# atom501/v-img

Measured on AMD Instinct MI355X. Metric: Mrays/sec (primary+secondary) at 512 spp, higher is better.
Workload: dtype f32; 1 GPU; disney_spheres.json, mis integrator, 512 spp, 1800x800; integrator=mis, spp=512, depth=unbounded, bvh=sweep SAH (host)

## Files before the change

v-img_amd/csrc/hip_internal.h:

```cpp
#pragma once
#include <hip/hip_runtime.h>

#include <algorithm>
#include <string>
#include <utility>
#include <vector>

#include "../../include/vimg_hip.h"
#include "device_mem.h"
#include "device_scene.h"
#include "kernel_tus.h"

#pragma GCC visibility push(hidden)
struct VimgDeviceScene {
  vimg::DScene d{};
  vimg::DevBuf nodes, leaf_prims;
  vimg::DevBuf chain_leaf;
  std::vector<vimg::DevBuf> tables;
  size_t total_bytes = 0;
  bool textured = false;
  VimgHipOptions opt{};
  int waves_per_simd = 2;
  bool too_wide = false;
  bool force_general = false;
  bool no_lds_tables = false;
  uint32_t num_cus = 0;
  uint32_t num_leaf_prims = 0;
  vimg::DevBuf stats;
  vimg::DevBuf counter;
  vimg::DevBuf root_box;
  vimg::DevBuf frame;
  vimg::DevBuf pool_cold;
  vimg::DevBuf stack_ovf;
  vimg::DevBuf pool_state;
  uint32_t pool_epoch = 0;
  uint64_t generation = 0;
  uint32_t num_vertices = 0, num_tris = 0, num_spheres = 0;
  uint32_t num_meshes = 0;
  std::vector<std::pair<uint32_t, uint32_t>> normal_rows;
  uint32_t n_internal = 0;
// ... 111 lines not shown
};
int enqueue_render(VimgDeviceScene* s, const VimgRenderParams* p, const RenderLaunch& r);
int check_kernel_error(VimgDeviceScene* s);
uint64_t fetch_shard_pixels(const VimgDeviceScene* s, const VimgRenderParams* p);
int fetch_stats(VimgDeviceScene* s, const VimgRenderParams* p, VimgRenderStats* out);

LaunchCfg make_launch(const VimgDeviceScene* s, const VimgRenderParams* p, int sx, int sy);
LaunchCfg make_launch_lane(const VimgDeviceScene* s, const VimgRenderParams* p, int sx, int sy);
LaunchCfg make_launch_feature(const VimgDeviceScene* s, const VimgRenderParams* p, int sx, int sy);
RenderArgs base_args(const VimgDeviceScene* s, const VimgRenderParams* p, int sx, int sy);
uint32_t segments_for(const VimgDeviceScene* s, const VimgRenderParams* p, uint64_t items, uint64_t in_flight,
                      double per_gen, double most, RenderArgs* a);
const void* kernel_of(const VimgDeviceScene* s, const LaunchCfg& c);
const void* launched_kernel_of(const VimgDeviceScene* s, const LaunchCfg& c, bool stats);
bool plain_launch_serves(const VimgDeviceScene* s, const LaunchCfg& c, bool stats);
void drop_unread_tables(const VimgDeviceScene* s, LaunchCfg& c, bool stats);

}
#pragma GCC visibility pop
```

v-img_amd/csrc/kernel_tus.h:

```cpp
#pragma once
#include "device_scene.h"

namespace vimg {

struct CuKArgs;
using RenderKernel = void (*)(const DScene, const RenderArgs, float*, DeviceStats*, unsigned int*);
using CuKernel = void (*)(const CuKArgs);

RenderKernel vimg_lane_kernel(bool tex, int wps);
RenderKernel vimg_feature_kernel(bool tex);
CuKernel vimg_cu_kernel(bool tex, bool deep, int nw);
CuKernel vimg_cu_kernel_early(bool tex, bool deep, int nw);
CuKernel vimg_cu_kernel_diag(bool tex, bool deep, int nw);
CuKernel vimg_cu_kernel_plain();
CuKernel vimg_cu_kernel_plain_early();

}
```

v-img_amd/csrc/launch_policy.hip:

```cpp
#include <cmath>

#include "hip_internal.h"
#include "render_cu_kernel.h"

namespace vimg {

uint32_t local_tiles(const VimgDeviceScene* s, const VimgRenderParams* p) {
  const uint32_t total = tiles_of(s->d.res_x) * tiles_of(s->d.res_y);
  if (p->tile_rank >= total) return 0;
  return (total - p->tile_rank + p->tile_world - 1) / p->tile_world;
}

RenderArgs base_args(const VimgDeviceScene* s, const VimgRenderParams* p, int sx, int sy) {
  const VimgHipOptions& o = s->opt;
  RenderArgs a{};
  a.integrator = p->integrator;
  a.samples = p->samples;
  a.spp_div = static_cast<float>(p->samples);
  a.depth = p->depth;
  a.tile_rank = p->tile_rank;
  a.tile_world = p->tile_world;
  a.tiles_x = tiles_of(s->d.res_x);
  a.tiles_y = tiles_of(s->d.res_y);
  a.num_local_tiles = local_tiles(s, p);
// ... 15 lines not shown
  const double gens = double(items) / double(in_flight);
  uint32_t k = gens >= 10.0 ? 1u : uint32_t(std::min(most, std::max(1.0, std::floor(per_gen / gens + 0.5))));
  k = std::min<uint32_t>(k, std::max<uint32_t>(p->samples / 4u, 1u));
  if (items * 2u < in_flight * 3u) k = 1u;
  if (s->opt.pool_segments != VIMG_OPT_AUTO) k = uint32_t(std::max(1, s->opt.pool_segments));
  k = std::min<uint32_t>(k, 4096u);
  while (k > 1u && items * k >= 0xfff00000ull) --k;
  const uint32_t len = std::max<uint32_t>((p->samples + k - 1) / k, 1u);
  a->pool_seg_len = len;
  a->pool_segments = std::max<uint32_t>((p->samples + len - 1) / len, 1u);
  return len;
}

namespace {

CuKernel pick_cu_kernel(const VimgDeviceScene* s, bool deep, int nw, bool diag = false, bool early = false, bool plain = false) {
  if (plain) return early ? vimg_cu_kernel_plain_early() : vimg_cu_kernel_plain();
  return diag ? vimg_cu_kernel_diag(s->textured, deep, nw)
              : (early ? vimg_cu_kernel_early(s->textured, deep, nw) : vimg_cu_kernel(s->textured, deep, nw));
}

void magic_div(uint32_t d, uint32_t* magic, uint32_t* shift) {
  uint32_t l = 0;
  while ((1ull << l) < d) ++l;
  *magic = static_cast<uint32_t>((1ull << (31u + l)) / d + 1ull);
  *shift = l - 1u;
}

constexpr uint32_t CU_LDS_LIMIT = 160u * 1024u;

LaunchCfg cu_launch_with(const VimgDeviceScene* s, const VimgRenderParams* p, int sx, int sy, uint32_t node_budget, uint32_t stack_cap) {
  LaunchCfg c{};
// ... 130 lines not shown
void cu_scratch(const VimgDeviceScene* s, LaunchCfg& c) {
  const RenderArgs& a = c.args;
  c.cold_bytes = size_t(c.grid) * cu_cold_records(s->textured) * a.pool_slots * 16u;
  if (a.stack_lds < a.stack_entries)
    c.ovf_bytes = size_t(c.grid) * a.cu_walkers * (a.stack_entries - a.stack_lds) * 256u;
}

}

const void* kernel_of(const VimgDeviceScene* s, const LaunchCfg& c) {
  if (c.feature) return reinterpret_cast<const void*>(vimg_feature_kernel(s->textured));
  if (c.sched == VIMG_SCHED_CU) return reinterpret_cast<const void*>(pick_cu_kernel(s, c.deep, c.cu_waves));
  return reinterpret_cast<const void*>(vimg_lane_kernel(s->textured, c.wps));
}

bool plain_launch_serves(const VimgDeviceScene* s, const LaunchCfg& c, bool stats) {
  return plain_build_serves(plain_launch_of(c.sched == VIMG_SCHED_CU, s->textured, c.deep, c.cu_waves, stats, s->force_general, c.args)) &&
         plain_tables_serve(c.args.lds_tables) && plain_leaf_perm_serves(c.args.leaf_perm);
}

void drop_unread_tables(const VimgDeviceScene* s, LaunchCfg& c, bool stats) {
  if (c.sched != VIMG_SCHED_CU || (c.args.lds_tables == 0u && c.args.leaf_perm == 0u) || plain_launch_serves(s, c, stats)) return;
  c.lds_bytes -= c.table_bytes;
  c.table_bytes = 0u;
  c.args.lds_tables = 0u;
  c.args.leaf_perm = 0u, c.args.leaf_perm_off = 0u, c.args.leaf_perm_stride = 0u;
}

const void* launched_kernel_of(const VimgDeviceScene* s, const LaunchCfg& c, bool stats) {
  if (c.sched != VIMG_SCHED_CU) return kernel_of(s, c);
  return reinterpret_cast<const void*>(pick_cu_kernel(s, c.deep, c.cu_waves, stats, (c.args.cu_flex & 32u) != 0u,
                                                      plain_launch_serves(s, c, stats)));
}

namespace {

LaunchCfg lane_shaped_launch(const VimgDeviceScene* s, const VimgRenderParams* p, int sx, int sy, bool feature) {
  LaunchCfg c{};
  c.feature = feature;
  const VimgHipOptions& o = s->opt;
  const uint64_t items = (sx >= 0) ? 1 : uint64_t(local_tiles(s, p)) * 64u;
  c.sched = VIMG_SCHED_LANE;
  c.wps = s->waves_per_simd;
  if (o.waves_per_simd != VIMG_OPT_AUTO) c.wps = o.waves_per_simd >= 3 ? 3 : 2;
  RenderArgs& a = c.args = base_args(s, p, sx, sy);
  a.stack_lds = a.stack_entries;
  const uint32_t stack_bytes = 4u * a.stack_entries * 64u * 4u;
// ... 62 lines not shown
```

v-img_amd/csrc/plain_build.h:

```cpp
#pragma once
#include <cstdint>

namespace vimg {

enum : uint32_t {
  PF_INTEGRATOR = 1u,
  PF_CLASSES = 2u,
  PF_LEAF_LDS = 4u,
  PF_SINGLE = 8u,
  PF_ITEMS = 16u,
  PF_FLEX = 32u,
  PF_TAB_HIT = 64u,
  PF_TAB_MAT = 128u,
  PF_TABLES = PF_TAB_HIT | PF_TAB_MAT,
  PF_LEAF_PERM = 256u,
};
#ifdef VIMG_PLAIN_FOLD
constexpr uint32_t PLAIN_FOLD = VIMG_PLAIN_FOLD;
#else
constexpr uint32_t PLAIN_FOLD = PF_INTEGRATOR | PF_CLASSES | PF_LEAF_LDS | PF_SINGLE | PF_ITEMS | PF_FLEX | PF_TAB_HIT | PF_LEAF_PERM;
#endif

struct PlainLaunch {
  bool cu_sched;
  bool textured, deep;
  int cu_waves;
  bool stats;
  bool force_general;
  uint32_t integrator, pool_classes, lds_leaf, cu_flex;
  int single_x;
  bool has_item_list;
};
constexpr uint32_t PLAIN_INTEGRATOR_MIS = 3u;
constexpr uint32_t PLAIN_FLEX_DEFAULT = 1u;

constexpr bool plain_build_serves(const PlainLaunch& l, uint32_t fold = PLAIN_FOLD) {
  if (l.force_general || !l.cu_sched || l.textured || l.deep || l.cu_waves != 16 || l.stats) return false;
  if ((fold & PF_INTEGRATOR) && l.integrator != PLAIN_INTEGRATOR_MIS) return false;
  if ((fold & PF_CLASSES) && l.pool_classes != 3u) return false;
  if ((fold & PF_LEAF_LDS) && l.lds_leaf == 0u) return false;
  if ((fold & PF_SINGLE) && l.single_x >= 0) return false;
  if ((fold & PF_ITEMS) && l.has_item_list) return false;
  if ((fold & PF_FLEX) && (l.cu_flex & ~32u) != PLAIN_FLEX_DEFAULT) return false;
  return true;
}

constexpr bool plain_tables_serve(uint32_t staged, uint32_t fold = PLAIN_FOLD) {
  return (staged & fold & PF_TABLES) == (fold & PF_TABLES);
}

constexpr bool plain_leaf_perm_serves(uint32_t ready, uint32_t fold = PLAIN_FOLD) {
  return !(fold & PF_LEAF_PERM) || ready != 0u;
}

template <class Args>
constexpr PlainLaunch plain_launch_of(bool cu_sched, bool textured, bool deep, int cu_waves, bool stats, bool force_general,
                                      const Args& a) {
  return PlainLaunch{cu_sched, textured, deep, cu_waves, stats || a.full_stats != 0u, force_general,
                     a.integrator, a.pool_classes, a.lds_leaf, a.cu_flex, a.single_x, a.item_list != nullptr};
}

}
```

v-img_amd/csrc/render_cu_kernel.h:

```cpp
#pragma once
#include <type_traits>

#include "plain_build.h"
#include "render_kernels.h"

namespace vimg {

enum : uint32_t {
  SC_THROUGHPUT = 0,
  SC_RESULT,
  SC_NEE,
  SC4_RNG,
  SC4_MAIN
};
__host__ __device__ constexpr uint32_t cu_cold_records(bool tex) { return SC4_MAIN + 1u + (tex ? 1u : 0u); }
__host__ __device__ constexpr uint32_t cu_stack_rows_of(uint32_t entries, uint32_t in_lds) { return in_lds < entries ? in_lds + 1u : entries; }
constexpr uint32_t SLOT_IDLE = 0xffffffffu;

VD void state_store(VIMG_GLOBAL uint32_t* p, uint32_t v) {
  __hip_atomic_store(p, v, __ATOMIC_RELAXED, __HIP_MEMORY_SCOPE_AGENT);
}
VD uint32_t state_load(VIMG_GLOBAL uint32_t* p) {
  return __hip_atomic_load(p, __ATOMIC_RELAXED, __HIP_MEMORY_SCOPE_AGENT);
}
// ... 39 lines not shown
  unsigned long long w_cyc[4];
  unsigned long long wait_cyc[5], wait_n[5];
  unsigned long long ray_cyc, ray_n;
  unsigned long long pv_cyc[6], pv_n;
};
static_assert(sizeof(CuWaveRec) == 416, "CuWaveRec layout");
__host__ __device__ constexpr uint32_t cu_pool_bytes(uint32_t slots, uint32_t waves) {
  return CU_LDS_BYTES * slots + uint32_t(sizeof(CuCtl)) + waves * uint32_t(sizeof(CuWaveRec));
}
VD uint32_t cu_mod(uint32_t n, uint32_t d, uint32_t magic, uint32_t shift) { return n - d * (__umulhi(n, magic) >> shift); }
VD int32_t lds_add_rtn(VIMG_LDS int32_t* p, int32_t v) { return __hip_atomic_fetch_add(p, v, __ATOMIC_RELAXED, __HIP_MEMORY_SCOPE_WORKGROUP); }
VD uint32_t lds_add_rtn(VIMG_LDS uint32_t* p, uint32_t v) { return __hip_atomic_fetch_add(p, v, __ATOMIC_RELAXED, __HIP_MEMORY_SCOPE_WORKGROUP); }
VD uint32_t lds_load(VIMG_LDS uint32_t* p) { return __hip_atomic_load(p, __ATOMIC_RELAXED, __HIP_MEMORY_SCOPE_WORKGROUP); }
VD int32_t lds_load(VIMG_LDS int32_t* p) { return __hip_atomic_load(p, __ATOMIC_RELAXED, __HIP_MEMORY_SCOPE_WORKGROUP); }
VD uint32_t cu_uni(uint32_t v) { return static_cast<uint32_t>(__builtin_amdgcn_readfirstlane(static_cast<int>(v))); }

static_assert(PLAIN_INTEGRATOR_MIS == uint32_t(VIMG_INTEGRATOR_MIS), "plain_build.h");
template <uint32_t PLAIN> VD uint32_t opt_integrator(const RenderArgs& A) {
  if constexpr (PLAIN & PF_INTEGRATOR) return uint32_t(VIMG_INTEGRATOR_MIS); else return A.integrator;
}
template <uint32_t PLAIN> VD uint32_t opt_classes(const RenderArgs& A) {
  if constexpr (PLAIN & PF_CLASSES) return 3u; else return A.pool_classes;
}
template <uint32_t PLAIN> VD bool opt_leaf_in_lds(const RenderArgs& A) {
  if constexpr (PLAIN & PF_LEAF_LDS) return true; else return A.lds_leaf != 0u;
}
template <uint32_t PLAIN> VD bool opt_single(const RenderArgs& A) {
  if constexpr (PLAIN & PF_SINGLE) return false; else return A.single_x >= 0;
}
template <uint32_t PLAIN> VD bool opt_has_items(const RenderArgs& A) {
  if constexpr (PLAIN & PF_ITEMS) return false; else return A.item_list != nullptr;
}
template <uint32_t PLAIN> VD uint32_t opt_flex(const RenderArgs& A) {
  if constexpr (PLAIN & PF_FLEX) return PLAIN_FLEX_DEFAULT; else return A.cu_flex;
}
template <uint32_t PLAIN> constexpr bool opt_leaf_perm = (PLAIN & PF_LEAF_PERM) != 0u;

template <class T>
VD void stage_rows(VIMG_LDS unsigned char* lds_raw, const RenderArgs& A, uint32_t t, gptr<T> src) {
  constexpr uint32_t src_w = uint32_t(sizeof(T)) / 4u;
  const uint32_t dst_w = tab_row_bytes(t) / 4u, words = A.tab_rows[t] * src_w;
  VIMG_LDS uint32_t* dst = reinterpret_cast<VIMG_LDS uint32_t*>(lds_raw + A.tab_off[t]);
  gptr<uint32_t> w = reinterpret_cast<gptr<uint32_t>>(src);
  for (uint32_t i = threadIdx.x; i < words; i += blockDim.x) {
    const uint32_t r = i / src_w;
    dst[r * dst_w + (i - r * src_w)] = w[i];
  }
}
VD void stage_tables(const DScene& g, const RenderArgs& A, VIMG_LDS unsigned char* lds_raw) {
  if (A.lds_tables & PF_TAB_HIT) {
// ... 117 lines not shown
                                         \
  [[maybe_unused]] auto slot_complete = [&](uint32_t nw) -> bool {                                                      \
    return (nw & CF_DONE_V) && (!(nw & CF_HAS_S) || (nw & CF_DONE_S)) && (!(nw & CF_HAS_R) || (nw & CF_DONE_R));        \
  };                                                                                                                    \
    \
  [[maybe_unused]] auto hand_to_vertex = [&](bool complete, uint32_t nw, uint32_t slot_) {                              \
    uint32_t cls_ = 0;                                                                                                  \
    if (complete && (nw & CF_FOUND) && !(nw & CF_KILL_R) && opt_integrator<PLAIN>(A) >= VIMG_INTEGRATOR_MATERIAL) {     \
      cls_ = (nw >> CF_CLS_SHIFT) & 3u;                                                                                 \
      if (cls_ == 0 && material_mode) cls_ = 3;                            \
      if (cls_ != 0) {                                                                                                  \
        if (opt_classes<PLAIN>(A) == 1) cls_ = 1;                                                                       \
        else if (opt_classes<PLAIN>(A) == 2) cls_ = (cls_ == 2) ? 2u : 1u;                                              \
      }                                                                                                                 \
    }                                                                                                                   \
    const unsigned long long m0_ = __ballot(complete && cls_ == 0), m1_ = __ballot(complete && cls_ == 1),              \
                             m2_ = __ballot(complete && cls_ == 2), m3_ = __ballot(complete && cls_ == 3);              \
    if ((m0_ | m1_ | m2_ | m3_) == 0ull) return;                                                                        \
    const uint32_t n_me_ = static_cast<uint32_t>(__popcll(lane == 0 ? m0_ : (lane == 1 ? m1_ : (lane == 2 ? m2_ : m3_)))); \
    uint32_t t_me_ = 0;                                                                                                 \
    if (lane < 4u && n_me_ != 0u) {                                                                                     \
      t_me_ = lds_add_rtn(&G->tail[lane], n_me_);                                                                       \
      if (t_me_ > 0x7ff00000u) raise(8u);                                                                               \
    }                                                                                                                   \
    const uint32_t t0_ = __shfl(t_me_, 0), t1_ = __shfl(t_me_, 1), t2_ = __shfl(t_me_, 2), t3_ = __shfl(t_me_, 3);      \
    if (complete) {                                                                                                     \
      const uint32_t tt_ = cls_ == 0 ? t0_ : (cls_ == 1 ? t1_ : (cls_ == 2 ? t2_ : t3_));                               \
      const unsigned long long mm_ = cls_ == 0 ? m0_ : (cls_ == 1 ? m1_ : (cls_ == 2 ? m2_ : m3_));                     \
      *ring_at(cls_, tt_ + lane_rank(mm_, lane)) = static_cast<uint16_t>(slot_);                                        \
      if (full_stats) tq[slot_] = static_cast<uint32_t>(__builtin_readcyclecounter());                                  \
    }                                                                                                                   \
    __builtin_amdgcn_fence(__ATOMIC_RELEASE, "workgroup");                                                              \
    if (lane < 4u && n_me_ != 0u) lds_add_rtn(&G->avail[lane], static_cast<int32_t>(n_me_));                            \
  };                                                                                                                    \
                     \
  [[maybe_unused]] auto push_rays = [&](bool is_s, bool is_r, uint32_t slot_) {                                         \
    const unsigned long long ms_ = __ballot(is_s), mr_ = __ballot(is_r);                                                \
    const uint32_t n_s_ = static_cast<uint32_t>(__popcll(ms_)), n_r_ = static_cast<uint32_t>(__popcll(mr_));            \
    if (n_s_ + n_r_ == 0u) return;                                                                                      \
    uint32_t t_ = 0;                                                                                                    \
    if (lane == 0) {                                                                                                    \
      t_ = lds_add_rtn(&G->tail[CQ_WALK], n_s_ + n_r_);                                                                 \
      if (t_ > 0x7ff00000u) raise(8u);                                                                                  \
    }                                                                                                                   \
    t_ = cu_uni(t_);                                                                                                    \
    if (is_s) *ring_at(CQ_WALK, t_ + lane_rank(ms_, lane)) = static_cast<uint16_t>(slot_ | CU_RAY_S);                   \
    if (is_r) *ring_at(CQ_WALK, t_ + n_s_ + lane_rank(mr_, lane)) = static_cast<uint16_t>(slot_);                       \
    __builtin_amdgcn_fence(__ATOMIC_RELEASE, "workgroup");                                                              \
// ... 672 lines not shown
        const float root = slab(load3k(g.root_min), load3k(g.root_max), ray.o, w_inv, ray.min_t, ray.max_t);
        cur = is_inf(root) ? REF_DONE : g.root_ref;
        sp = 0;
        w_found = false;
        rec.prim = 0xffffffffu;
        w_setup = false;
      }
    }
    wlap(wc0);
    if (__ballot(w_slot != SLOT_IDLE) == 0ull) break;

    const bool exact_round = __any(w_exact && w_slot != SLOT_IDLE);
    for (;;) {
      auto box_loop = [&](auto exact_possible) {
        for (;;) {
          const bool act = cur != REF_DONE && ref_count(cur) == 0;
          if (!__any(act)) break;
          if (full_stats) d_box += 1u, d_boxl += static_cast<uint32_t>(__popcll(__ballot(act)));
          if (act) {
            v4f na, nb, nc;
            v2u refs;
            if (!DEEP || cur < L.n_nodes) {
              na = L.na[cur], nb = L.nb[cur], nc = L.nc[cur];
              refs = L.nm[cur];
            } else {
              gptr<DNode> nd = g.nodes + cur;
              na = nd->a, nb = nd->b, nc = nd->c;
              refs = v2u{nd->left_ref, nd->right_ref};
            }
            const uint32_t sp_below = sp != 0 ? sp - 1 : 0u;
            uint32_t popped = stack0[(DEEP ? (sp_below < S ? sp_below : S) : sp_below) * 64];
            c_internal += stat_inc;
            float h1, h2;
            if (decltype(exact_possible)::value && w_exact) {
// ... 3 lines not shown
              h1 = slab_fast(f3{na.x, na.y, na.z}, f3{na.w, nb.x, nb.y}, ray.o, w_inv, ray.min_t, ray.max_t);
              h2 = slab_fast(f3{nb.z, nb.w, nc.x}, f3{nc.y, nc.z, nc.w}, ray.o, w_inv, ray.min_t, ray.max_t);
            }
            const bool in1 = !is_inf(h1), in2 = !is_inf(h2);
            const uint32_t c1 = refs.x, c2 = refs.y;
            const bool both = in1 && in2, any = in1 || in2;
            const bool first_is_near = w_any ? false : (h2 > h1);
            const uint32_t near_c = first_is_near ? c1 : c2;
            const uint32_t far_c = first_is_near ? c2 : c1;
            stack0[(DEEP ? (sp < S ? sp : S) : sp) * 64] = far_c;
            if constexpr (DEEP) {
              if (both && sp >= S) ovf0[(sp - S) * 64] = far_c;
              if (!any && sp_below >= S) popped = ovf0[(sp_below - S) * 64];
            }
            const uint32_t one_c = in1 ? c1 : c2;
            cur = both ? near_c : (any ? one_c : (sp != 0 ? popped : REF_DONE));
            sp = both ? sp + 1 : (any ? sp : sp_below);
          }
          if constexpr (DEEP) {
            if (static_cast<uint32_t>(__popcll(__ballot(cur != REF_DONE && ref_count(cur) == 0))) < box_min) break;
          }
        }
      };
      if (exact_round)
        box_loop(std::true_type{});
      else
        box_loop(std::false_type{});
      wlap(wc1);

      if (full_stats) d_leaf += 1u, d_leafl += static_cast<uint32_t>(__popcll(__ballot(cur != REF_DONE && (!DEEP || ref_count(cur) != 0))));
      if (cur != REF_DONE && (!DEEP || ref_count(cur) != 0)) {
        const uint32_t first = ref_index(cur), count = ref_count(cur);
        c_leaf += stat_inc;
        bool stop = false;
        [[maybe_unused]] const VIMG_LDS v4f* leaf0 =
// ... 32 lines not shown
          rec.e2 = keep_rec ? e2 : rec.e2, rec.inv_det = keep_rec ? idet : rec.inv_det;
          rec.prim = keep_rec ? lp_prim : rec.prim;
          rec.kind = keep_rec ? kind : rec.kind;
          w_cls = keep_rec ? lp_cls : w_cls;
          stop = hit && w_any;
        }
        const uint32_t sp_below = sp != 0 ? sp - 1 : 0u;
        uint32_t popped = stack0[(DEEP ? (sp_below < S ? sp_below : S) : sp_below) * 64];
        if constexpr (DEEP) {
          if (!stop && sp_below >= S) popped = ovf0[(sp_below - S) * 64];
        }
        cur = (stop || sp == 0) ? REF_DONE : popped;
        sp = sp_below;
      }
      wlap(wc2);
      const uint32_t n_fin = static_cast<uint32_t>(__popcll(__ballot(w_slot != SLOT_IDLE && cur == REF_DONE)));
      const uint32_t n_act = static_cast<uint32_t>(__popcll(__ballot(w_slot != SLOT_IDLE && cur != REF_DONE)));
      if (n_act == 0 || n_fin >= A.pool_refill) break;
    }

    {
      const bool done = w_slot != SLOT_IDLE && cur == REF_DONE;
      bool complete = false;
      uint32_t nw = 0;
      if (done) {
        uint32_t orv;
        if (w_type == 0u) {
          orv = CF_DONE_S | (w_found ? CF_OCCLUDED : 0u);
        } else {
          orv = CF_DONE_R;
          if (w_found) {
            orv |= CF_FOUND | (rec.kind == 1 ? CF_KIND_SPHERE : 0u) | (w_cls << CF_CLS_SHIFT);
            wr(CR_HIT, w_slot, v4u{fu(rec.e0), fu(rec.e1), fu(rec.e2), fu(rec.inv_det)});
// ... 67 lines not shown
  uint32_t polls = 0;
  unsigned long long idle_since = 0;
  for (;;) {
    const CuKPtr K = cu_kargs();
    CU_STAGE_LOCALS(K);
    auto lap = [&](uint32_t k) {
      if (full_stats) {
        const unsigned long long now = __builtin_readcyclecounter();
        if (lane == 0) wrec->cyc[k] += now - t_mark;
        t_mark = now;
      }
    };
    if (cu_uni(lds_load(&G->abort)) != 0u) break;
    const v4u av4 = *reinterpret_cast<VIMG_LDS v4u*>(&G->avail[0]);
    const int32_t a0 = skip_fin ? 0 : static_cast<int32_t>(cu_uni(av4.x)), a1 = static_cast<int32_t>(cu_uni(av4.y)),
                  a2 = static_cast<int32_t>(cu_uni(av4.z)), a3 = static_cast<int32_t>(cu_uni(av4.w));
    const int32_t aw = static_cast<int32_t>(cu_uni(static_cast<uint32_t>(lds_load(&G->avail[CQ_WALK]))));
    const int32_t m01 = a0 > a1 ? a0 : a1, m23 = a2 > a3 ? a2 : a3, qmax = m01 > m23 ? m01 : m23;
    if (full_stats && lane == 0) {
      wrec->looks += 1;
      wrec->q_sum[0] += static_cast<uint32_t>(a0 > 0 ? a0 : 0), wrec->q_sum[1] += static_cast<uint32_t>(a1 > 0 ? a1 : 0);
      wrec->q_sum[2] += static_cast<uint32_t>(a2 > 0 ? a2 : 0), wrec->q_sum[3] += static_cast<uint32_t>(aw > 0 ? aw : 0);
    }
    if (can_walk && aw > 0 && (aw >= static_cast<int32_t>(A.cu_join) || polls >= A.cu_patience)) {
      lap(5);
      skip_fin = false, polls = 0, idle_since = 0;
      if (full_stats) iter_wave++;
      if (opt_flex<PLAIN>(A) & 4u) __builtin_amdgcn_s_setprio(1);
      cu_walk<TEX, DEEP, NW, DIAG, PLAIN>(n_closest, n_shadow);
      if (opt_flex<PLAIN>(A) & 4u) __builtin_amdgcn_s_setprio(0);
      lap(4);
// ... 12 lines not shown
      lap(5);
      if (full_stats) iter_wave++;
      if (full_stats && lane == 0) wrec->nbatch[cls] += 1, wrec->nslots[cls] += n;
      if (full_stats) {
        unsigned long long w = lane < n ? static_cast<unsigned long long>(static_cast<uint32_t>(__builtin_readcyclecounter()) - tq[e]) : 0ull;
        for (int o = 32; o; o >>= 1) w += __shfl_xor(w, o);
        if (lane == 0) wrec->wait_cyc[cls] += w, wrec->wait_n[cls] += n;
      }
      bool all_pending = false;
      const bool by_class = opt_classes<PLAIN>(A) == 3u;
      if (opt_flex<PLAIN>(A) & 2u) __builtin_amdgcn_s_setprio(1);
      if (cls == 0u)
        cu_vertex<TEX, NW, DIAG, EARLY, true, -1, PLAIN>(n, e, all_pending, n_nan, n_dead);
      else if (cls == 1u && by_class)
        cu_vertex<TEX, NW, DIAG, EARLY, false, int(VIMG_MAT_LAMBERTIAN), PLAIN>(n, e, all_pending, n_nan, n_dead);
      else if (cls == 2u && by_class)
        cu_vertex<TEX, NW, DIAG, EARLY, false, int(VIMG_MAT_PRINCIPLED), PLAIN>(n, e, all_pending, n_nan, n_dead);
      else
        cu_vertex<TEX, NW, DIAG, EARLY, false, -1, PLAIN>(n, e, all_pending, n_nan, n_dead);
      if (opt_flex<PLAIN>(A) & 2u) __builtin_amdgcn_s_setprio(0);
      skip_fin = all_pending;
      if (!all_pending) polls = 0, idle_since = 0;
      lap(cls);
      continue;
    }
    if (cu_uni(lds_load(&G->live)) == 0u) break;
    skip_fin = false;
    polls += 1;
    if ((polls & 255u) == 0u) {
      const unsigned long long now = __builtin_amdgcn_s_memrealtime();
      if (idle_since == 0) idle_since = now;
      else if (static_cast<uint32_t>((now - idle_since) >> 20) > A.cu_watchdog) {
        if (lane == 0) raise(1u);
// ... 45 lines not shown
```

v-img_amd/csrc/render_kernels.h:

```cpp
#pragma once
#include "device_math.h"
#include "device_scene.h"
#include "material_terms.h"
#include "plain_build.h"

namespace vimg {


struct Rng {
  uint64_t s;
};
VD uint32_t pcg_next(Rng& r) {
  uint64_t old = r.s;
  r.s = old * 6364136223846793005ULL + 1ULL;
  uint32_t xorshifted = static_cast<uint32_t>(((old >> 18u) ^ old) >> 27u);
  uint32_t rot = static_cast<uint32_t>(old >> 59u);
  return (xorshifted >> rot) | (xorshifted << ((0u - rot) & 31u));
}
VD void pcg_seed(Rng& r, uint64_t initstate) {
  r.s = 0;
  pcg_next(r);
  r.s += initstate;
  pcg_next(r);
}
// ... 354 lines not shown
  f3 p2t = tri_vertex<PERMUTED>(p2, o, rc.kz);
  p0t.x += rc.sx * p0t.z;
  p0t.y += rc.sy * p0t.z;
  p1t.x += rc.sx * p1t.z;
  p1t.y += rc.sy * p1t.z;
  p2t.x += rc.sx * p2t.z;
  p2t.y += rc.sy * p2t.z;
  float e0 = diff_of_products(p1t.x, p2t.y, p1t.y, p2t.x);
  float e1 = diff_of_products(p2t.x, p0t.y, p2t.y, p0t.x);
  float e2 = diff_of_products(p0t.x, p1t.y, p0t.y, p1t.x);
  if (e0 == 0.f || e1 == 0.f || e2 == 0.f) {
    e0 = diff_of_products_double(p1t.x, p2t.y, p1t.y, p2t.x);
    e1 = diff_of_products_double(p2t.x, p0t.y, p2t.y, p0t.x);
    e2 = diff_of_products_double(p0t.x, p1t.y, p0t.y, p1t.x);
  }
  const bool mixed = (e0 < 0 || e1 < 0 || e2 < 0) && (e0 > 0 || e1 > 0 || e2 > 0);
  const float det = e0 + e1 + e2;
  const float t_scaled = e0 * (p0t.z * rc.sz) + e1 * (p1t.z * rc.sz) + e2 * (p2t.z * rc.sz);
  const float hi = ray.max_t * det, lo = ray.min_t * det;
  const bool out_neg = det < 0 && (t_scaled >= 0 || t_scaled < hi || t_scaled > lo);
  const bool out_pos = det > 0 && (t_scaled <= 0 || t_scaled > hi || t_scaled < lo);
  const bool hit = !mixed && !(det == 0) && !out_neg && !out_pos;
  if (hit) {
    const float inv_det = 1.f / det;
    t_out = t_scaled * inv_det;
    e0o = e0, e1o = e1, e2o = e2, inv_det_o = inv_det;
  }
  return hit;
}
VD bool tri_test_flat(f3 p0, f3 p1, f3 p2, const TravRay& ray, const TriRayConst& rc, float& t_out,
                      float& e0o, float& e1o, float& e2o, float& inv_det_o) {
  return tri_test_body<false>(p0, p1, p2, ray.o, ray, rc, t_out, e0o, e1o, e2o, inv_det_o);
}
VD bool tri_test_permuted(f3 p0, f3 p1, f3 p2, f3 o_perm, const TravRay& ray, const TriRayConst& rc, float& t_out,
                          float& e0o, float& e1o, float& e2o, float& inv_det_o) {
  return tri_test_body<true>(p0, p1, p2, o_perm, ray, rc, t_out, e0o, e1o, e2o, inv_det_o);
}
// ... 1431 lines not shown
```

v-img_amd/csrc/scene_bake.h:

```cpp
#pragma once
#include "device_scene.h"

namespace vimg {

#define VHD static __host__ __device__ __forceinline__

VHD void tri_cross21(const float* v, float c21[3]) {
  const float e1[3] = {v[3] - v[0], v[4] - v[1], v[5] - v[2]};
  const float e2[3] = {v[6] - v[0], v[7] - v[1], v[8] - v[2]};
  c21[0] = e2[1] * e1[2] - e1[1] * e2[2];
  c21[1] = e2[2] * e1[0] - e1[2] * e2[0];
  c21[2] = e2[0] * e1[1] - e1[0] * e2[1];
}

VHD void bake_tri_normal_pdf(const float* v, float n[3], float* area_pdf) {
  const float e1[3] = {v[3] - v[0], v[4] - v[1], v[5] - v[2]};
  const float e2[3] = {v[6] - v[0], v[7] - v[1], v[8] - v[2]};
  const float c12[3] = {e1[1] * e2[2] - e2[1] * e1[2], e1[2] * e2[0] - e2[2] * e1[0],
                        e1[0] * e2[1] - e2[0] * e1[1]};
  const float inv_len = 1.0f / __builtin_sqrtf(c12[0] * c12[0] + c12[1] * c12[1] + c12[2] * c12[2]);
  for (int a = 0; a < 3; ++a) n[a] = c12[a] * inv_len;
  float c21[3];
  tri_cross21(v, c21);
  const float area = __builtin_sqrtf(c21[0] * c21[0] + c21[1] * c21[1] + c21[2] * c21[2]) / 2.0f;
// ... 14 lines not shown
}

VHD void bake_light_tri(const DTriShade& ts, float area_pdf, DLight& L) {
  L.a = v4f{ts.p[0], ts.p[1], ts.p[2], ts.p[3]};
  L.b = v4f{ts.p[4], ts.p[5], ts.p[6], ts.p[7]};
  L.c = v4f{ts.p[8], ts.n[0], ts.n[1], ts.n[2]};
  L.d.w = area_pdf;
}
VHD void bake_light_sphere(const VimgSphere& sp, DLight& L) {
  L.a = v4f{sp.center[0], sp.center[1], sp.center[2], sp.radius};
}

VHD uint32_t bake_material_class(uint32_t type) {
  return type == VIMG_MAT_DIFFUSE_LIGHT ? 0u : type == VIMG_MAT_LAMBERTIAN ? 1u : type == VIMG_MAT_PRINCIPLED ? 2u : 3u;
}
VHD uint32_t bake_material_flags(const VimgMaterial& m, const VimgTexture* textures) {
  uint32_t f = 0;
  if (m.type == VIMG_MAT_PRINCIPLED) f |= MATF_NEEDS_FRAME;
  if (m.tex >= 0 && textures[m.tex].type != VIMG_TEX_CONST) f |= MATF_NEEDS_UV;
  if (m.mr_tex >= 0 || m.normal_map >= 0) f |= MATF_NEEDS_UV;
  return f;
}
VHD uint32_t bake_prim_material(const VimgPrim& p, const DTriShade* shade, const VimgMesh* meshes, const VimgSphere* spheres) {
  return p.type == VIMG_PRIM_TRIANGLE ? meshes[shade[p.index].mesh].material : spheres[p.index].material;
}
VHD DLight bake_light(const VimgLight& l, const VimgPrim* prims, const DTriShade* shade, const float* area_pdf, const VimgMesh* meshes,
                      const VimgSphere* spheres, const VimgMaterial* materials) {
  DLight L{};
  if (l.type == VIMG_LIGHT_BACKGROUND) {
    L.kind = 0u;
// ... 31 lines not shown
```

v-img_amd/csrc/scene_relight.hip:

```cpp
#include <hip/hip_runtime.h>

#include <cstring>

#include "device_math.h"
#include "hip_internal.h"
#include "material_terms.h"
#include "scene_bake.h"

namespace vimg {

namespace {

constexpr uint32_t kBlock = 256;

template <typename T>
VD T* flat(gptr<T> p) {
  return (T*)p;
}

dim3 blocks_for(uint32_t n) { return dim3((n + kBlock - 1) / kBlock); }

}

__global__ void __launch_bounds__(kBlock) scene_relight_flags(const DScene d, uint32_t num_materials) {
// ... 149 lines not shown
      HIP_TRY(hipMemcpyAsync(plan->new_lights.p, u->lights, size_t(u->num_lights) * sizeof(VimgLight), hipMemcpyHostToDevice, st));
      hipLaunchKernelGGL(scene_relight_lights, blocks_for(u->num_lights), dim3(kBlock), 0, st, d, plan->new_lights.as<const VimgLight>(),
                         u->num_lights, plan->new_dlights.as<DLight>());
    }
  } else if (u->materials && d.num_lights) {
    hipLaunchKernelGGL(scene_relight_lights, blocks_for(d.num_lights), dim3(kBlock), 0, st, d, (const VimgLight*)d.lights, d.num_lights,
                       (DLight*)d.dlights);
  }
  HIP_TRY(hipGetLastError());
  return VIMG_OK;
}

void commit_relight(VimgDeviceScene* s, const VimgGeometryUpdate* u, RelightPlan* plan) {
  DScene& d = s->d;
  if (u->textures) s->textures.assign(u->textures, u->textures + s->textures.size());
  if (u->materials) s->materials.assign(u->materials, u->materials + s->materials.size());
  if (u->background) {
    d.background = *u->background;
    d.background_emissive = background_is_emissive(d.background);
  }
  if (plan->new_dmaterials.p) {
    DevBuf& dmaterials = s->tables[s->dmaterials_table];
    dmaterials = std::move(plan->new_dmaterials);
    d.dmaterials = (decltype(d.dmaterials))dmaterials.p;
  }
  s->textured = tables_textured(s->materials.data(), static_cast<uint32_t>(s->materials.size()), s->textures.data(), d.background);
  if (u->set_lights) {
    DevBuf& lights = s->tables[s->lights_table];
    DevBuf& dlights = s->tables[s->dlights_table];
    s->total_bytes = s->total_bytes - lights.bytes - dlights.bytes + plan->new_lights.bytes + plan->new_dlights.bytes;
    lights = std::move(plan->new_lights);
// ... 11 lines not shown
```

v-img_amd/csrc/scene_upload.hip:

```cpp
#include <cmath>
#include <cstdlib>
#include <cstring>
#include <memory>
#include <numbers>

#include "hip_internal.h"
#include "scene_bake.h"
#include "scene_update.h"

using namespace vimg;

namespace {

template <typename T>
int upload(VimgDeviceScene* s, DevBuf& b, const T* host, size_t count) {
  if (int rc = b.alloc(std::max<size_t>(count, 1) * sizeof(T))) return rc;
  s->total_bytes += b.bytes;
  if (count) HIP_TRY(hipMemcpy(b.p, host, count * sizeof(T), hipMemcpyHostToDevice));
  return VIMG_OK;
}

}

int vimg::validate_materials(const VimgMaterial* materials, uint32_t num_materials, const VimgTexture* textures, uint32_t num_textures,
// ... 359 lines not shown
    s->total_bytes += b.bytes;
    s->dmaterials_table = s->tables.size() - 1;
    d.dmaterials = (decltype(d.dmaterials))b.p;
    if (int rc = enqueue_material_bake(d, sc->num_materials, b.as<DMaterial>(), nullptr)) return rc;
    HIP_TRY(hipStreamSynchronize(nullptr));
  }
  if (!t.chain_leaf.empty()) {
    if (int rc = s->chain_leaf.alloc(t.chain_leaf.size() * sizeof(uint32_t))) return rc;
    HIP_TRY(hipMemcpy(s->chain_leaf.p, t.chain_leaf.data(), s->chain_leaf.bytes, hipMemcpyHostToDevice));
  }
  return VIMG_OK;
}

void record_for_updates(VimgDeviceScene* s, const VimgScene* sc) {
  s->materials.assign(sc->materials, sc->materials + sc->num_materials);
  s->textures.assign(sc->textures, sc->textures + sc->num_textures);
  s->lights.assign(sc->lights, sc->lights + sc->num_lights);
  s->num_rg_textures = sc->num_rg_textures;
  s->num_texels = sc->num_texels;
  s->num_cdf = sc->num_cdf;
  s->num_vertices = sc->num_vertices;
  s->num_tris = sc->num_tris;
  s->num_spheres = sc->num_spheres;
  s->num_meshes = sc->num_meshes;
  for (uint32_t i = 0; i < sc->num_meshes; ++i) {
    const VimgMesh& m = sc->meshes[i];
    if (!m.has_normals || m.num_vertices == 0) continue;
    auto& r = s->normal_rows;
    if (!r.empty() && r.back().first + r.back().second == m.first_vertex)
      r.back().second += m.num_vertices;
// ... 151 lines not shown
```

v-img_amd/csrc/vimg_hip.hip:

```cpp
#include <cstdio>
#include <cstdlib>
#include <memory>

#include "hip_internal.h"
#include "aux_kernels.h"
#include "render_cu_kernel.h"
#include "heatmap_kernel.h"

namespace vimg {

hipStream_t g_stream = nullptr;
int g_device = -1;

namespace {
thread_local std::string g_err;
}

int fail(int code, const std::string& msg) {
  g_err = msg;
  return code;
}

}

// ... 351 lines not shown
  for (auto& e : ev)
    if (int rc2 = e.create()) return rc2;
  for (int i = 0; i < steps; ++i) {
    if (int rc2 = enqueue_render(s, p, {.d_out = static_cast<float*>(d_out), .st = g_stream, .ev0 = ev[2 * i].e, .ev1 = ev[2 * i + 1].e}))
      return rc2;
  }
  HIP_TRY(hipStreamSynchronize(g_stream));
  if (int rc2 = check_kernel_error(s)) return rc2;
  for (int i = 0; i < steps; ++i) HIP_TRY(hipEventElapsedTime(&ms_per_launch[i], ev[2 * i].e, ev[2 * i + 1].e));
  return VIMG_OK;
}

int vimg_hip_probe(VimgDeviceScene* s, int kind, int n, const float* in_host, float* out_host) {
  static const int n_in[11] = {0, 4, 6, 7, 12, 8, 4, 5, 1, 8, 12};
  static const int n_out[11] = {0, 8, 28, 1, 5, 7, 10, 4, 5, 8, 8};
  if (!s || kind < 1 || kind > 10 || n <= 0 || !in_host || !out_host)
    return fail(VIMG_E_INVALID, "probe: bad arguments");
  DevBuf d_in, d_out;
  if (int rc = d_in.alloc(size_t(n) * n_in[kind] * sizeof(float))) return rc;
  if (int rc = d_out.alloc(size_t(n) * n_out[kind] * sizeof(float))) return rc;
  HIP_TRY(hipMemcpy(d_in.p, in_host, size_t(n) * n_in[kind] * sizeof(float), hipMemcpyHostToDevice));
  VimgRenderParams p{VIMG_INTEGRATOR_MIS, 1, 1, 0, 1};
  LaunchCfg c = make_launch_lane(s, &p, -1, -1);
  const uint32_t grid = (uint32_t(n) + 255) / 256;
  if (s->textured)
    hipLaunchKernelGGL(probe_kernel<true>, dim3(grid), dim3(256), c.lds_bytes, g_stream, s->d, c.args,
                       kind, n, d_in.as<float>(), d_out.as<float>());
  else
    hipLaunchKernelGGL(probe_kernel<false>, dim3(grid), dim3(256), c.lds_bytes, g_stream, s->d, c.args,
                       kind, n, d_in.as<float>(), d_out.as<float>());
// ... 8 lines not shown
```

v-img_amd/hip.py:

```python
import ctypes as C

import numpy as np

from . import _abi as abi
from .host import HostScene, camera_lookat, make_params


PROBE_IO = {1: (4, 8), 2: (6, 28), 3: (7, 1), 4: (12, 5), 5: (8, 7), 6: (4, 10), 7: (5, 4), 8: (1, 5), 9: (8, 8), 10: (12, 8)}


class HipError(RuntimeError):
    pass


def _lib():
    return abi.hip_lib()


def _checker(lib, last_error):
    def check(rc):
        if rc < 0:
            raise HipError(f"[{rc}] " + getattr(lib(), last_error)().decode())
        return rc
    return check
# ... 216 lines not shown
                             if v.textures[i].type == abi.TEX_IMAGE}
        self.camera = abi.Camera.from_buffer_copy(v.camera)
        self.generation = 0
        self.vertices_given, self.spheres_given = None, None

    @property
    def bytes(self):
        return int(self._lib.vimg_hip_scene_bytes(self._h))

    @property
    def kernel(self):
        return self._lib.vimg_hip_scene_kernel(self._h).decode()

    def kernel_for(self, params):
        return self._lib.vimg_hip_launch_kernel(self._h, C.byref(params)).decode()

    def shard_pixels(self, params):
        return _check(self._lib.vimg_hip_shard_pixels(self._h, C.byref(params)))

    def render(self, params, out=None, stats=True, stream=None):
        c = _Tensors()
        out = c.own(self._new_output(params)) if out is None else c.use(out)
        st = abi.RenderStats()
        with c.launch(stream) as sp:
            _check(self._lib.vimg_hip_render(self._h, C.byref(params), C.c_void_p(out.data_ptr()), sp,
                                             C.byref(st) if stats else None))
        return (out, st) if stats else out

    def render_features(self, params, features=("albedo", "normal", "depth"), out=None, stream=None):
        unknown = [f for f in features if f not in abi.FEATURES]
# ... 536 lines not shown
```

Baseline: 15790 Mrays/s.

## Specialize plain CU kernel for scenes without 'other' material class

Adds a PF_NO_OTHER fold bit, set on the host when no material falls in class 3. With it, the plain kernel drops the fourth queue ballot and atomic, ignores its avail counter, and routes everything to the principled vertex path, so the generic material path is not compiled in. A second plain kernel variant without the bit is built for scenes that do use other materials. It also keeps the box-loop active mask in scalar registers via ballot/inverse_ballot and turns the triangle test's short-circuit logic into bitwise ops to cut branching. The cost is extra kernel instantiations and more selection logic.

```diff
diff --git a/v-img_amd/csrc/hip_internal.h b/v-img_amd/csrc/hip_internal.h
--- a/v-img_amd/csrc/hip_internal.h
+++ b/v-img_amd/csrc/hip_internal.h
@@ -24,6 +24,7 @@
   bool too_wide = false;
   bool force_general = false;
   bool no_lds_tables = false;
+  bool has_other = false;
   uint32_t num_cus = 0;
   uint32_t num_leaf_prims = 0;
   vimg::DevBuf stats;
@@ -165,6 +166,7 @@
 const void* kernel_of(const VimgDeviceScene* s, const LaunchCfg& c);
 const void* launched_kernel_of(const VimgDeviceScene* s, const LaunchCfg& c, bool stats);
 bool plain_launch_serves(const VimgDeviceScene* s, const LaunchCfg& c, bool stats);
+uint32_t plain_fold_of(const VimgDeviceScene* s, const LaunchCfg& c, bool stats);
 void drop_unread_tables(const VimgDeviceScene* s, LaunchCfg& c, bool stats);
 
 }
diff --git a/v-img_amd/csrc/k_cu_plain_other.hip b/v-img_amd/csrc/k_cu_plain_other.hip
--- /dev/null
+++ b/v-img_amd/csrc/k_cu_plain_other.hip
@@ -0,0 +1,6 @@
+#include "kernel_tus.h"
+#include "render_cu_kernel.h"
+
+namespace vimg {
+CuKernel vimg_cu_kernel_plain_other() { return render_cu_kernel<false, false, 16, 4, false, 0, PLAIN_FOLD_OTHER>; }
+}
diff --git a/v-img_amd/csrc/k_cu_plain_other_early.hip b/v-img_amd/csrc/k_cu_plain_other_early.hip
--- /dev/null
+++ b/v-img_amd/csrc/k_cu_plain_other_early.hip
@@ -0,0 +1,6 @@
+#include "kernel_tus.h"
+#include "render_cu_kernel.h"
+
+namespace vimg {
+CuKernel vimg_cu_kernel_plain_other_early() { return render_cu_kernel<false, false, 16, 4, false, 1, PLAIN_FOLD_OTHER>; }
+}
diff --git a/v-img_amd/csrc/kernel_tus.h b/v-img_amd/csrc/kernel_tus.h
--- a/v-img_amd/csrc/kernel_tus.h
+++ b/v-img_amd/csrc/kernel_tus.h
@@ -14,5 +14,7 @@
 CuKernel vimg_cu_kernel_diag(bool tex, bool deep, int nw);
 CuKernel vimg_cu_kernel_plain();
 CuKernel vimg_cu_kernel_plain_early();
+CuKernel vimg_cu_kernel_plain_other();
+CuKernel vimg_cu_kernel_plain_other_early();
 
 }
diff --git a/v-img_amd/csrc/launch_policy.hip b/v-img_amd/csrc/launch_policy.hip
--- a/v-img_amd/csrc/launch_policy.hip
+++ b/v-img_amd/csrc/launch_policy.hip
@@ -53,8 +53,9 @@
 
 namespace {
 
-CuKernel pick_cu_kernel(const VimgDeviceScene* s, bool deep, int nw, bool diag = false, bool early = false, bool plain = false) {
-  if (plain) return early ? vimg_cu_kernel_plain_early() : vimg_cu_kernel_plain();
+CuKernel pick_cu_kernel(const VimgDeviceScene* s, bool deep, int nw, bool diag = false, bool early = false, uint32_t plain = 0u) {
+  if (plain == PLAIN_FOLD) return early ? vimg_cu_kernel_plain_early() : vimg_cu_kernel_plain();
+  if (plain != 0u) return early ? vimg_cu_kernel_plain_other_early() : vimg_cu_kernel_plain_other();
   return diag ? vimg_cu_kernel_diag(s->textured, deep, nw)
               : (early ? vimg_cu_kernel_early(s->textured, deep, nw) : vimg_cu_kernel(s->textured, deep, nw));
 }
@@ -215,10 +216,12 @@
   return reinterpret_cast<const void*>(vimg_lane_kernel(s->textured, c.wps));
 }
 
-bool plain_launch_serves(const VimgDeviceScene* s, const LaunchCfg& c, bool stats) {
-  return plain_build_serves(plain_launch_of(c.sched == VIMG_SCHED_CU, s->textured, c.deep, c.cu_waves, stats, s->force_general, c.args)) &&
-         plain_tables_serve(c.args.lds_tables) && plain_leaf_perm_serves(c.args.leaf_perm);
-}
+uint32_t plain_fold_of(const VimgDeviceScene* s, const LaunchCfg& c, bool stats) {
+  if (!plain_tables_serve(c.args.lds_tables) || !plain_leaf_perm_serves(c.args.leaf_perm)) return 0u;
+  return plain_fold_serving(plain_launch_of(c.sched == VIMG_SCHED_CU, s->textured, c.deep, c.cu_waves, stats, s->force_general, c.args,
+                                            s->has_other));
+}
+bool plain_launch_serves(const VimgDeviceScene* s, const LaunchCfg& c, bool stats) { return plain_fold_of(s, c, stats) != 0u; }
 
 void drop_unread_tables(const VimgDeviceScene* s, LaunchCfg& c, bool stats) {
   if (c.sched != VIMG_SCHED_CU || (c.args.lds_tables == 0u && c.args.leaf_perm == 0u) || plain_launch_serves(s, c, stats)) return;
@@ -231,7 +234,7 @@
 const void* launched_kernel_of(const VimgDeviceScene* s, const LaunchCfg& c, bool stats) {
   if (c.sched != VIMG_SCHED_CU) return kernel_of(s, c);
   return reinterpret_cast<const void*>(pick_cu_kernel(s, c.deep, c.cu_waves, stats, (c.args.cu_flex & 32u) != 0u,
-                                                      plain_launch_serves(s, c, stats)));
+                                                      plain_fold_of(s, c, stats)));
 }
 
 namespace {
diff --git a/v-img_amd/csrc/plain_build.h b/v-img_amd/csrc/plain_build.h
--- a/v-img_amd/csrc/plain_build.h
+++ b/v-img_amd/csrc/plain_build.h
@@ -14,12 +14,14 @@
   PF_TAB_MAT = 128u,
   PF_TABLES = PF_TAB_HIT | PF_TAB_MAT,
   PF_LEAF_PERM = 256u,
+  PF_NO_OTHER = 512u,
 };
 #ifdef VIMG_PLAIN_FOLD
 constexpr uint32_t PLAIN_FOLD = VIMG_PLAIN_FOLD;
 #else
-constexpr uint32_t PLAIN_FOLD = PF_INTEGRATOR | PF_CLASSES | PF_LEAF_LDS | PF_SINGLE | PF_ITEMS | PF_FLEX | PF_TAB_HIT | PF_LEAF_PERM;
+constexpr uint32_t PLAIN_FOLD = PF_INTEGRATOR | PF_CLASSES | PF_LEAF_LDS | PF_SINGLE | PF_ITEMS | PF_FLEX | PF_TAB_HIT | PF_LEAF_PERM | PF_NO_OTHER;
 #endif
+constexpr uint32_t PLAIN_FOLD_OTHER = PLAIN_FOLD & ~PF_NO_OTHER;
 
 struct PlainLaunch {
   bool cu_sched;
@@ -30,6 +32,7 @@
   uint32_t integrator, pool_classes, lds_leaf, cu_flex;
   int single_x;
   bool has_item_list;
+  bool has_other = false;
 };
 constexpr uint32_t PLAIN_INTEGRATOR_MIS = 3u;
 constexpr uint32_t PLAIN_FLEX_DEFAULT = 1u;
@@ -42,7 +45,11 @@
   if ((fold & PF_SINGLE) && l.single_x >= 0) return false;
   if ((fold & PF_ITEMS) && l.has_item_list) return false;
   if ((fold & PF_FLEX) && (l.cu_flex & ~32u) != PLAIN_FLEX_DEFAULT) return false;
+  if ((fold & PF_NO_OTHER) && l.has_other) return false;
   return true;
+}
+constexpr uint32_t plain_fold_serving(const PlainLaunch& l) {
+  return plain_build_serves(l, PLAIN_FOLD) ? PLAIN_FOLD : (plain_build_serves(l, PLAIN_FOLD_OTHER) ? PLAIN_FOLD_OTHER : 0u);
 }
 
 constexpr bool plain_tables_serve(uint32_t staged, uint32_t fold = PLAIN_FOLD) {
@@ -55,9 +62,9 @@
 
 template <class Args>
 constexpr PlainLaunch plain_launch_of(bool cu_sched, bool textured, bool deep, int cu_waves, bool stats, bool force_general,
-                                      const Args& a) {
+                                      const Args& a, bool has_other = false) {
   return PlainLaunch{cu_sched, textured, deep, cu_waves, stats || a.full_stats != 0u, force_general,
-                     a.integrator, a.pool_classes, a.lds_leaf, a.cu_flex, a.single_x, a.item_list != nullptr};
+                     a.integrator, a.pool_classes, a.lds_leaf, a.cu_flex, a.single_x, a.item_list != nullptr, has_other};
 }
 
 }
diff --git a/v-img_amd/csrc/render_cu_kernel.h b/v-img_amd/csrc/render_cu_kernel.h
--- a/v-img_amd/csrc/render_cu_kernel.h
+++ b/v-img_amd/csrc/render_cu_kernel.h
@@ -77,6 +77,12 @@
 VD uint32_t lds_load(VIMG_LDS uint32_t* p) { return __hip_atomic_load(p, __ATOMIC_RELAXED, __HIP_MEMORY_SCOPE_WORKGROUP); }
 VD int32_t lds_load(VIMG_LDS int32_t* p) { return __hip_atomic_load(p, __ATOMIC_RELAXED, __HIP_MEMORY_SCOPE_WORKGROUP); }
 VD uint32_t cu_uni(uint32_t v) { return static_cast<uint32_t>(__builtin_amdgcn_readfirstlane(static_cast<int>(v))); }
+VD unsigned long long cu_mask(bool p) {
+  unsigned long long m = __builtin_amdgcn_ballot_w64(p);
+  asm volatile("" : "+s"(m));
+  return m;
+}
+VD bool cu_lanes(unsigned long long m) { return __builtin_amdgcn_inverse_ballot_w64(m); }
 
 static_assert(PLAIN_INTEGRATOR_MIS == uint32_t(VIMG_INTEGRATOR_MIS), "plain_build.h");
 template <uint32_t PLAIN> VD uint32_t opt_integrator(const RenderArgs& A) {
@@ -97,6 +103,8 @@
 template <uint32_t PLAIN> VD uint32_t opt_flex(const RenderArgs& A) {
   if constexpr (PLAIN & PF_FLEX) return PLAIN_FLEX_DEFAULT; else return A.cu_flex;
 }
+template <uint32_t PLAIN> constexpr bool opt_no_other =
+    (PLAIN & (PF_NO_OTHER | PF_INTEGRATOR | PF_CLASSES)) == (PF_NO_OTHER | PF_INTEGRATOR | PF_CLASSES);
 template <uint32_t PLAIN> constexpr bool opt_leaf_perm = (PLAIN & PF_LEAF_PERM) != 0u;
 
 template <class T>
@@ -244,24 +252,26 @@
         else if (opt_classes<PLAIN>(A) == 2) cls_ = (cls_ == 2) ? 2u : 1u;                                              \
       }                                                                                                                 \
     }                                                                                                                   \
+                            \
+    constexpr bool four_ = !opt_no_other<PLAIN>;                                                                        \
     const unsigned long long m0_ = __ballot(complete && cls_ == 0), m1_ = __ballot(complete && cls_ == 1),              \
-                             m2_ = __ballot(complete && cls_ == 2), m3_ = __ballot(complete && cls_ == 3);              \
+                             m2_ = __ballot(complete && cls_ == 2), m3_ = four_ ? __ballot(complete && cls_ == 3) : 0ull;\
     if ((m0_ | m1_ | m2_ | m3_) == 0ull) return;                                                                        \
-    const uint32_t n_me_ = static_cast<uint32_t>(__popcll(lane == 0 ? m0_ : (lane == 1 ? m1_ : (lane == 2 ? m2_ : m3_)))); \
+    const uint32_t n_me_ = static_cast<uint32_t>(__popcll(lane == 0 ? m0_ : (lane == 1 ? m1_ : ((!four_ || lane == 2) ? m2_ : m3_))));\
     uint32_t t_me_ = 0;                                                                                                 \
-    if (lane < 4u && n_me_ != 0u) {                                                                                     \
+    if (lane < (four_ ? 4u : 3u) && n_me_ != 0u) {                                                                      \
       t_me_ = lds_add_rtn(&G->tail[lane], n_me_);                                                                       \
       if (t_me_ > 0x7ff00000u) raise(8u);                                                                               \
     }                                                                                                                   \
-    const uint32_t t0_ = __shfl(t_me_, 0), t1_ = __shfl(t_me_, 1), t2_ = __shfl(t_me_, 2), t3_ = __shfl(t_me_, 3);      \
+    const uint32_t t0_ = __shfl(t_me_, 0), t1_ = __shfl(t_me_, 1), t2_ = __shfl(t_me_, 2), t3_ = four_ ? __shfl(t_me_, 3) : 0u;\
     if (complete) {                                                                                                     \
-      const uint32_t tt_ = cls_ == 0 ? t0_ : (cls_ == 1 ? t1_ : (cls_ == 2 ? t2_ : t3_));                               \
-      const unsigned long long mm_ = cls_ == 0 ? m0_ : (cls_ == 1 ? m1_ : (cls_ == 2 ? m2_ : m3_));                     \
+      const uint32_t tt_ = cls_ == 0 ? t0_ : (cls_ == 1 ? t1_ : ((!four_ || cls_ == 2) ? t2_ : t3_));                   \
+      const unsigned long long mm_ = cls_ == 0 ? m0_ : (cls_ == 1 ? m1_ : ((!four_ || cls_ == 2) ? m2_ : m3_));         \
       *ring_at(cls_, tt_ + lane_rank(mm_, lane)) = static_cast<uint16_t>(slot_);                                        \
       if (full_stats) tq[slot_] = static_cast<uint32_t>(__builtin_readcyclecounter());                                  \
     }                                                                                                                   \
     __builtin_amdgcn_fence(__ATOMIC_RELEASE, "workgroup");                                                              \
-    if (lane < 4u && n_me_ != 0u) lds_add_rtn(&G->avail[lane], static_cast<int32_t>(n_me_));                            \
+    if (lane < (four_ ? 4u : 3u) && n_me_ != 0u) lds_add_rtn(&G->avail[lane], static_cast<int32_t>(n_me_));                            \
   };                                                                                                                    \
                      \
   [[maybe_unused]] auto push_rays = [&](bool is_s, bool is_r, uint32_t slot_) {                                         \
@@ -964,10 +974,10 @@
     for (;;) {
       auto box_loop = [&](auto exact_possible) {
         for (;;) {
-          const bool act = cur != REF_DONE && ref_count(cur) == 0;
-          if (!__any(act)) break;
-          if (full_stats) d_box += 1u, d_boxl += static_cast<uint32_t>(__popcll(__ballot(act)));
-          if (act) {
+          const unsigned long long m_act = cu_mask(cur != REF_DONE && ref_count(cur) == 0);
+          if (m_act == 0ull) break;
+          if (full_stats) d_box += 1u, d_boxl += static_cast<uint32_t>(__popcll(m_act));
+          if (cu_lanes(m_act)) {
             v4f na, nb, nc;
             v2u refs;
             if (!DEEP || cur < L.n_nodes) {
@@ -1001,11 +1011,13 @@
               if (!any && sp_below >= S) popped = ovf0[(sp_below - S) * 64];
             }
             const uint32_t one_c = in1 ? c1 : c2;
-            cur = both ? near_c : (any ? one_c : (sp != 0 ? popped : REF_DONE));
-            sp = both ? sp + 1 : (any ? sp : sp_below);
+            const uint32_t pop_c = sp != 0 ? popped : REF_DONE;
+            const uint32_t part_c = any ? one_c : pop_c, part_sp = any ? sp : sp_below;
+            cur = both ? near_c : part_c;
+            sp = both ? sp + 1 : part_sp;
           }
           if constexpr (DEEP) {
-            if (static_cast<uint32_t>(__popcll(__ballot(cur != REF_DONE && ref_count(cur) == 0))) < box_min) break;
+            if (static_cast<uint32_t>(__popcll(__builtin_amdgcn_ballot_w64(cur != REF_DONE && ref_count(cur) == 0))) < box_min) break;
           }
         }
       };
@@ -1068,9 +1080,8 @@
         sp = sp_below;
       }
       wlap(wc2);
-      const uint32_t n_fin = static_cast<uint32_t>(__popcll(__ballot(w_slot != SLOT_IDLE && cur == REF_DONE)));
-      const uint32_t n_act = static_cast<uint32_t>(__popcll(__ballot(w_slot != SLOT_IDLE && cur != REF_DONE)));
-      if (n_act == 0 || n_fin >= A.pool_refill) break;
+      const uint32_t n_fin = static_cast<uint32_t>(__popcll(__builtin_amdgcn_ballot_w64(w_slot != SLOT_IDLE && cur == REF_DONE)));
+      if (__builtin_amdgcn_ballot_w64(w_slot != SLOT_IDLE && cur != REF_DONE) == 0ull || n_fin >= A.pool_refill) break;
     }
 
     {
@@ -1168,7 +1179,7 @@
     if (cu_uni(lds_load(&G->abort)) != 0u) break;
     const v4u av4 = *reinterpret_cast<VIMG_LDS v4u*>(&G->avail[0]);
     const int32_t a0 = skip_fin ? 0 : static_cast<int32_t>(cu_uni(av4.x)), a1 = static_cast<int32_t>(cu_uni(av4.y)),
-                  a2 = static_cast<int32_t>(cu_uni(av4.z)), a3 = static_cast<int32_t>(cu_uni(av4.w));
+                  a2 = static_cast<int32_t>(cu_uni(av4.z)), a3 = opt_no_other<PLAIN> ? 0 : static_cast<int32_t>(cu_uni(av4.w));
     const int32_t aw = static_cast<int32_t>(cu_uni(static_cast<uint32_t>(lds_load(&G->avail[CQ_WALK]))));
     const int32_t m01 = a0 > a1 ? a0 : a1, m23 = a2 > a3 ? a2 : a3, qmax = m01 > m23 ? m01 : m23;
     if (full_stats && lane == 0) {
@@ -1211,9 +1222,9 @@
         cu_vertex<TEX, NW, DIAG, EARLY, true, -1, PLAIN>(n, e, all_pending, n_nan, n_dead);
       else if (cls == 1u && by_class)
         cu_vertex<TEX, NW, DIAG, EARLY, false, int(VIMG_MAT_LAMBERTIAN), PLAIN>(n, e, all_pending, n_nan, n_dead);
-      else if (cls == 2u && by_class)
+      else if ((cls == 2u && by_class) || opt_no_other<PLAIN>)
         cu_vertex<TEX, NW, DIAG, EARLY, false, int(VIMG_MAT_PRINCIPLED), PLAIN>(n, e, all_pending, n_nan, n_dead);
-      else
+      else if constexpr (!opt_no_other<PLAIN>)
         cu_vertex<TEX, NW, DIAG, EARLY, false, -1, PLAIN>(n, e, all_pending, n_nan, n_dead);
       if (opt_flex<PLAIN>(A) & 2u) __builtin_amdgcn_s_setprio(0);
       skip_fin = all_pending;
diff --git a/v-img_amd/csrc/render_kernels.h b/v-img_amd/csrc/render_kernels.h
--- a/v-img_amd/csrc/render_kernels.h
+++ b/v-img_amd/csrc/render_kernels.h
@@ -392,13 +392,13 @@
     e1 = diff_of_products_double(p2t.x, p0t.y, p2t.y, p0t.x);
     e2 = diff_of_products_double(p0t.x, p1t.y, p0t.y, p1t.x);
   }
-  const bool mixed = (e0 < 0 || e1 < 0 || e2 < 0) && (e0 > 0 || e1 > 0 || e2 > 0);
+  const bool mixed = ((e0 < 0) | (e1 < 0) | (e2 < 0)) & ((e0 > 0) | (e1 > 0) | (e2 > 0));
   const float det = e0 + e1 + e2;
   const float t_scaled = e0 * (p0t.z * rc.sz) + e1 * (p1t.z * rc.sz) + e2 * (p2t.z * rc.sz);
   const float hi = ray.max_t * det, lo = ray.min_t * det;
-  const bool out_neg = det < 0 && (t_scaled >= 0 || t_scaled < hi || t_scaled > lo);
-  const bool out_pos = det > 0 && (t_scaled <= 0 || t_scaled > hi || t_scaled < lo);
-  const bool hit = !mixed && !(det == 0) && !out_neg && !out_pos;
+  const bool out_neg = (det < 0) & ((t_scaled >= 0) | (t_scaled < hi) | (t_scaled > lo));
+  const bool out_pos = (det > 0) & ((t_scaled <= 0) | (t_scaled > hi) | (t_scaled < lo));
+  const bool hit = !(mixed | (det == 0) | out_neg | out_pos);
   if (hit) {
     const float inv_det = 1.f / det;
     t_out = t_scaled * inv_det;
diff --git a/v-img_amd/csrc/scene_bake.h b/v-img_amd/csrc/scene_bake.h
--- a/v-img_amd/csrc/scene_bake.h
+++ b/v-img_amd/csrc/scene_bake.h
@@ -52,6 +52,11 @@
 VHD uint32_t bake_material_class(uint32_t type) {
   return type == VIMG_MAT_DIFFUSE_LIGHT ? 0u : type == VIMG_MAT_LAMBERTIAN ? 1u : type == VIMG_MAT_PRINCIPLED ? 2u : 3u;
 }
+inline bool table_holds_other(const VimgMaterial* materials, size_t n) {
+  for (size_t i = 0; i < n; ++i)
+    if (bake_material_class(materials[i].type) == 3u) return true;
+  return false;
+}
 VHD uint32_t bake_material_flags(const VimgMaterial& m, const VimgTexture* textures) {
   uint32_t f = 0;
   if (m.type == VIMG_MAT_PRINCIPLED) f |= MATF_NEEDS_FRAME;
diff --git a/v-img_amd/csrc/scene_relight.hip b/v-img_amd/csrc/scene_relight.hip
--- a/v-img_amd/csrc/scene_relight.hip
+++ b/v-img_amd/csrc/scene_relight.hip
@@ -187,7 +187,10 @@
 void commit_relight(VimgDeviceScene* s, const VimgGeometryUpdate* u, RelightPlan* plan) {
   DScene& d = s->d;
   if (u->textures) s->textures.assign(u->textures, u->textures + s->textures.size());
-  if (u->materials) s->materials.assign(u->materials, u->materials + s->materials.size());
+  if (u->materials) {
+    s->materials.assign(u->materials, u->materials + s->materials.size());
+    s->has_other = table_holds_other(s->materials.data(), s->materials.size());
+  }
   if (u->background) {
     d.background = *u->background;
     d.background_emissive = background_is_emissive(d.background);
diff --git a/v-img_amd/csrc/scene_upload.hip b/v-img_amd/csrc/scene_upload.hip
--- a/v-img_amd/csrc/scene_upload.hip
+++ b/v-img_amd/csrc/scene_upload.hip
@@ -397,6 +397,7 @@
 
 void record_for_updates(VimgDeviceScene* s, const VimgScene* sc) {
   s->materials.assign(sc->materials, sc->materials + sc->num_materials);
+  s->has_other = table_holds_other(s->materials.data(), s->materials.size());
   s->textures.assign(sc->textures, sc->textures + sc->num_textures);
   s->lights.assign(sc->lights, sc->lights + sc->num_lights);
   s->num_rg_textures = sc->num_rg_textures;
diff --git a/v-img_amd/csrc/vimg_hip.hip b/v-img_amd/csrc/vimg_hip.hip
--- a/v-img_amd/csrc/vimg_hip.hip
+++ b/v-img_amd/csrc/vimg_hip.hip
@@ -389,6 +389,17 @@
 int vimg_hip_probe(VimgDeviceScene* s, int kind, int n, const float* in_host, float* out_host) {
   static const int n_in[11] = {0, 4, 6, 7, 12, 8, 4, 5, 1, 8, 12};
   static const int n_out[11] = {0, 8, 28, 1, 5, 7, 10, 4, 5, 8, 8};
+  if (s && kind == 11 && n > 0 && in_host && out_host) {
+    for (int i = 0; i < n; ++i) {
+      const float* v = in_host + size_t(i) * 5;
+      const VimgRenderParams p{uint32_t(v[0]), uint32_t(v[1]), uint32_t(v[2]), uint32_t(v[3]), uint32_t(v[4])};
+      out_host[i] = 0.f;
+      if (p.tile_world == 0 || p.tile_rank >= p.tile_world || is_feature_integrator(p.integrator)) continue;
+      const LaunchCfg c = make_launch(s, &p, -1, -1);
+      if (!c.error && c.sched == VIMG_SCHED_CU) out_host[i] = float(plain_fold_of(s, c, false));
+    }
+    return VIMG_OK;
+  }
   if (!s || kind < 1 || kind > 10 || n <= 0 || !in_host || !out_host)
     return fail(VIMG_E_INVALID, "probe: bad arguments");
   DevBuf d_in, d_out;
diff --git a/v-img_amd/hip.py b/v-img_amd/hip.py
--- a/v-img_amd/hip.py
+++ b/v-img_amd/hip.py
@@ -6,7 +6,8 @@
 from .host import HostScene, camera_lookat, make_params
 
 
-PROBE_IO = {1: (4, 8), 2: (6, 28), 3: (7, 1), 4: (12, 5), 5: (8, 7), 6: (4, 10), 7: (5, 4), 8: (1, 5), 9: (8, 8), 10: (12, 8)}
+PROBE_IO = {1: (4, 8), 2: (6, 28), 3: (7, 1), 4: (12, 5), 5: (8, 7), 6: (4, 10), 7: (5, 4), 8: (1, 5), 9: (8, 8), 10: (12, 8), 11: (5, 1)}
+PROBE_LAUNCH_BUILD = 11
 
 
 class HipError(RuntimeError):
@@ -254,6 +255,10 @@
 
     def kernel_for(self, params):
         return self._lib.vimg_hip_launch_kernel(self._h, C.byref(params)).decode()
+
+    def plain_fold_for(self, params):
+        p = params
+        return int(self.probe(PROBE_LAUNCH_BUILD, [[p.integrator, p.samples, p.depth & 0xFFFFFF, p.tile_rank, p.tile_world]])[0, 0])
 
     def shard_pixels(self, params):
         return _check(self._lib.vimg_hip_shard_pixels(self._h, C.byref(params)))
```

After: 16070 Mrays/s, median of 6. 1.02x the previous value.
